# gnlpfjh/Scalable-E3-GNN

Measured on AMD Instinct MI355X. Metric: particles/sec (octree build + SEGNN fwd), 1M pts l_max=2, 1/2/4/8 MI355X, higher is better.
Workload: dtype f32; 1 GPU; 1000000 particles/GPU uniform in unit box, radius graph k~24 (E=23519616), SEGNN l_max=2 4 layers H=32 f32 storage; particles_per_gpu=1000000, edges_per_gpu=23519616, hidden=32, layers=4, lmax=2, parallelism=single GPU

## Files before the change

### include/e3gnn.h

```cpp
#ifndef E3GNN_H
#define E3GNN_H

#include <stdint.h>

#ifdef __cplusplus
extern "C" {
#endif

#define E3GNN_ABI_VERSION 3

enum {
  E3_OK = 0,
  E3_ERR_INVALID_ARG = 1,
  E3_ERR_BAD_IRREPS = 2,
  E3_ERR_MISSING_WEIGHT = 3,
  E3_ERR_UNSUPPORTED = 4,
  E3_ERR_HIP = 5,
  E3_ERR_NO_DEVICE = 6
};

enum { E3_F32 = 0, E3_F64 = 1, E3_BF16 = 2 };

enum { E3_CLS_0E = 0, E3_CLS_0O = 1, E3_CLS_1E = 2, E3_CLS_1O = 3 };

// ... 107 lines not shown
                       int dtype, void* packed, void* stream);
int e3_tp_forward(const e3_tp_plan* plan, const void* in1, int64_t ld_in1, const void* in2, int64_t ld_in2,
                  const void* packed, void* out, int64_t ld_out, int64_t B, int dtype, const float* in_scale,
                  int exact, void* stream);
int e3_pow2_scale(const e3_tp_segment* segs, const int64_t* nrows, int nseg, int target_log2, float* out4,
                  void* stream);
int e3_add_pow2_scale(const float* h, const float* u, float* out, int64_t n, int target_log2, float* out4,
                      void* stream);
int e3_tp_forward_fused(const e3_tp_plan* plan, const e3_tp_segment* segs, int nseg,
                        const void* in2, int64_t ld_in2, const void* packed, void* out, int64_t ld_out,
                        int64_t B, int dtype, int gate, const float* in_scale, void* stream);
int e3_tp_forward_fused_epilogue(const e3_tp_plan* plan, const e3_tp_segment* segs, int nseg, const void* in2,
                                 int64_t ld_in2, const void* packed, void* out, int64_t ld_out, int64_t B, int dtype,
                                 int gate, const float* in_scale, const void* residual, int64_t ld_residual,
                                 float* out_scale4, int target_log2, void* stream);
int e3_tp_backward(const e3_tp_plan* plan, const void* in1, int64_t ld_in1, const void* in2, int64_t ld_in2,
                   const void* packed, const void* grad_out, int64_t ld_gout, void* grad_in1, int64_t ld_gin1,
                   void* grad_in2, int64_t ld_gin2, void* const grad_weights[6], int64_t B, int dtype, void* stream);
int e3_tp_backward_weights(const e3_tp_plan* plan, const void* in1, int64_t ld_in1, const void* in2, int64_t ld_in2,
                           const void* packed, const void* grad_out, int64_t ld_gout, void* const grad_weights[6],
                           int64_t B, int dtype, void* stream);
int e3_tp_backward_operands(const e3_tp_plan* plan, const void* in1, int64_t ld_in1, const void* in2, int64_t ld_in2,
                            const void* packed, const void* grad_out, int64_t ld_gout, void* const features[6],
                            void* const gout[6], int64_t B, int dtype, void* stream);
int e3_tp_backward_contract(const e3_tp_plan* plan, const void* in1, int64_t ld_in1, const void* in2, int64_t ld_in2,
                            void* const t[6], void* grad_in1, int64_t ld_gin1, void* grad_in2, int64_t ld_gin2,
                            int64_t B, int dtype, void* stream);
int e3_tp_fused_supported(const e3_tp_plan* plan, int gate);
const char* e3_tp_last_fused_kernel(void);
int e3_tp_forward_fused_scatter(const e3_tp_plan* plan, const e3_tp_segment* segs, int nseg,
// ... 50 lines not shown
```

### scalable-e3-gnn_amd/_lib.py

```python
from __future__ import annotations

import ctypes
import os
from ctypes import POINTER, c_char_p, c_int, c_int32, c_int64, c_void_p

_HERE = os.path.dirname(os.path.abspath(__file__))
LIB_PATH = os.path.join(_HERE, "lib", "libe3gnn_hip.so")

E3_OK = 0
E3_F32, E3_F64, E3_BF16 = 0, 1, 2
CLS_NAMES = ("l0e", "l0o", "l1e", "l1o")

_lib = None

VoidP4 = c_void_p * 4
Float3 = ctypes.c_float * 3


class HaloEntry(ctypes.Structure):
    _fields_ = [("lo", ctypes.c_float * 3), ("hi", ctypes.c_float * 3), ("shift", ctypes.c_float * 3)]


SIGNATURES = {
    "e3_abi_version": (c_int, []),
# ... 71 lines not shown
    "e3_gate_blocks_backward": (c_int, [c_void_p, c_int64, c_void_p, c_int64, c_void_p, c_int64, c_int64, c_int, c_int,
                                        POINTER(c_int32), POINTER(c_int32), c_void_p]),
    "e3_segment_sum_backward": (c_int, [c_void_p, c_int64, c_void_p, c_int64, c_int, c_void_p, c_int64, c_void_p]),
    "e3_pow2_scale": (c_int, [c_void_p, POINTER(c_int64), c_int, c_int, c_void_p, c_void_p]),
    "e3_add_pow2_scale": (c_int, [c_void_p, c_void_p, c_void_p, c_int64, c_int, c_void_p, c_void_p]),
    "e3_tp_backward": (c_int, [c_void_p, c_void_p, c_int64, c_void_p, c_int64, c_void_p, c_void_p, c_int64, c_void_p,
                               c_int64, c_void_p, c_int64, c_void_p * 6, c_int64, c_int, c_void_p]),
    "e3_tp_backward_weights": (c_int, [c_void_p, c_void_p, c_int64, c_void_p, c_int64, c_void_p, c_void_p, c_int64, c_void_p,
                                       c_int64, c_int, c_void_p]),
    "e3_tp_backward_operands": (c_int, [c_void_p, c_void_p, c_int64, c_void_p, c_int64, c_void_p, c_void_p, c_int64, c_void_p,
                                        c_void_p, c_int64, c_int, c_void_p]),
    "e3_tp_backward_contract": (c_int, [c_void_p, c_void_p, c_int64, c_void_p, c_int64, c_void_p, c_void_p, c_int64, c_void_p,
                                        c_int64, c_int64, c_int, c_void_p]),
    "e3_tp_forward_fused_epilogue": (c_int, [c_void_p, c_void_p, c_int, c_void_p, c_int64, c_void_p, c_void_p, c_int64,
                                             c_int64, c_int, c_int, c_void_p, c_void_p, c_int64, c_void_p, c_int, c_void_p]),
    "e3_tp_fused_supported": (c_int, [c_void_p, c_int]),
    "e3_tp_last_fused_kernel": (ctypes.c_char_p, []),
    "e3_tp_forward_fused_scatter": (c_int, [c_void_p, c_void_p, c_int, c_void_p, c_int64, c_void_p, c_void_p, c_void_p,
                                            c_int64, c_int64, c_int, c_int, c_void_p, c_void_p]),
    "e3_segment_sum_bf16": (c_int, [c_void_p, c_int64, c_void_p, c_int64, c_int, c_void_p, c_int64, c_void_p]),
    "e3_edge_geometry_l2": (c_int, [c_void_p, c_void_p, c_void_p, c_int64, c_void_p, c_void_p, c_void_p, c_void_p]),
    "e3_gate_blocks": (c_int, [c_void_p, c_int64, c_void_p, c_int64, c_int64, c_int, c_int, POINTER(c_int32),
                               POINTER(c_int32), c_void_p]),
    "e3_l1tp_backward": (c_int, [c_void_p, c_void_p, c_int64, c_void_p, c_int64, VoidP4, VoidP4, c_void_p, c_int64,
                                 c_void_p, c_int64, c_void_p, VoidP4, c_void_p, c_int64, c_int, c_void_p]),
}


def load():
    global _lib
# ... 94 lines not shown
```

### scalable-e3-gnn_amd/csrc/e3_tp.hip

```cpp
#include "e3_common.h"
#include "cg_tables.h"
#include "e3_tp_internal.h"

#include <algorithm>
#include <cstdlib>
#include <map>
#include <mutex>
#include <utility>

namespace e3 {

static int tp_ensure_dyn_lds(const void* fn, size_t bytes) {
  if (bytes <= 64 * 1024) return E3_OK;
  static std::mutex mu;
  static std::map<std::pair<const void*, int>, size_t> have;
  int dev = 0;
  if (hipGetDevice(&dev) != hipSuccess) return E3_ERR_HIP;
  std::lock_guard<std::mutex> lock(mu);
  size_t& cur = have[std::make_pair(fn, dev)];
  if (bytes > cur) {
    if (hipFuncSetAttribute(fn, hipFuncAttributeMaxDynamicSharedMemorySize, (int)bytes) != hipSuccess) return E3_ERR_HIP;
    cur = bytes;
  }
  return E3_OK;
// ... 1112 lines not shown
  if ((dtype != E3_F32 && dtype != E3_BF16) || !plan->fast.usable || ld2 == 0) return E3_ERR_UNSUPPORTED;
  hipStream_t s = (hipStream_t)stream;
  if (out_scale4) E3_HIP_CHECK(hipMemsetAsync(out_scale4, 0, 16, s));
  if (B > 0) {
    if (!in2 || !packed || !out || ld2 < plan->dev.Dy) return E3_ERR_INVALID_ARG;
    int st = tp_ensure_device(plan);
    if (st != E3_OK) return st;
    st = fast_forward(&plan->fast, segs, nseg, plan->dev.D1, in2, ld2, (const char*)packed + fast_section_offset(plan), out,
                      ldo, B, gate, dtype, plan->dev.ocol, in_scale, s, nullptr, residual, ld_residual,
                      out_scale4 ? reinterpret_cast<uint32_t*>(out_scale4) + 2 : nullptr);
    if (st != E3_OK) return st;
  }
  return out_scale4 ? scale_finalize(out_scale4, target_log2, s) : E3_OK;
}

int e3_tp_forward_fused_scatter(const e3_tp_plan* plan, const e3_tp_segment* segs, int nseg, const void* in2,
                                int64_t ld2, const void* packed, const int32_t* row_node, void* out_nodes,
                                int64_t ldo, int64_t B, int dtype, int gate, const float* in_scale, void* stream) {
  if (!plan || !segs || !row_node || B < 0) return E3_ERR_INVALID_ARG;
  if ((dtype != E3_F32 && dtype != E3_BF16) || !gate || !plan->fast.usable || ld2 == 0) return E3_ERR_UNSUPPORTED;
  if (B == 0) return E3_OK;
  if (!in2 || !packed || !out_nodes || ld2 < plan->dev.Dy) return E3_ERR_INVALID_ARG;
  int st = tp_ensure_device(plan);
  if (st != E3_OK) return st;
  return fast_forward(&plan->fast, segs, nseg, plan->dev.D1, in2, ld2, (const char*)packed + fast_section_offset(plan),
                      out_nodes, ldo, B, gate, dtype, plan->dev.ocol, in_scale, (hipStream_t)stream, row_node);
}

int e3_tp_backward(const e3_tp_plan* plan, const void* in1, int64_t ld1, const void* in2, int64_t ld2,
                   const void* packed, const void* grad_out, int64_t ldg, void* grad_in1, int64_t ldg1,
// ... 100 lines not shown
```

### scalable-e3-gnn_amd/csrc/e3_tp_internal.h

```cpp
#pragma once
#include "e3_common.h"

#include <array>
#include <vector>

namespace e3 {

struct TpPath { int c1, l1, l2, wrow; };

struct FChunk {
  int col, count, l1;
  int wblk[3][3];
  int S[2], rows_per[2], inv[2];
};
struct FDev {
  int Dout, Dy, nchunks, ntab, lsh;
  int M[3], NT[3], Mpad[3], ooff[3];
  int bfoff[3];
  int bftotal;
};
struct FPack { int l3, orig_row, count, wblk; };

struct TpFast {
  FDev dev;
// ... 16 lines not shown
              const int32_t* ocol_tab, hipStream_t s);
int fast_forward(const TpFast* F, const e3_tp_segment* segs, int nseg, int D1, const void* in2, int64_t ld2,
                 const void* packed, void* out, int64_t ldo, int64_t B, int gate, int dtype, const int32_t* ocol_tab,
                 const float* in_scale, hipStream_t s, const int32_t* scatter = nullptr, const void* residual = nullptr,
                 int64_t ldr = 0, uint32_t* amax = nullptr);
int scale_finalize(float* out4, int target_log2, hipStream_t s);

void fast_note_kernel(const char* name);
const char* fast_last_kernel();

bool fast_gate_shape_ok(const TpFast* F);
bool r16_supported(const TpFast* F);
int fast_forward_r16(const TpFast* F, const void* seg_args, const void* in2, int64_t ld2, const void* packed, void* out,
                     int64_t ldo, int64_t B, int gate, int io16, const int32_t* ocol_tab, const float* in_scale,
                     hipStream_t s);

}
```

### scalable-e3-gnn_amd/csrc/e3_tp_mfma.hip

```cpp
#include "e3_common.h"
#include "e3_tp_internal.h"

#include <algorithm>
#include <cstdlib>
#include <vector>

namespace e3 {

#include "e3_tp_mfma_core.h"

template <typename T>
__global__ void fast_absmax_kernel(const T* w0, int64_t n0, const T* w1, int64_t n1, const T* w2, int64_t n2,
                                   uint32_t* hdr) {
  const T* w[3] = {w0, w1, w2};
  const int64_t n[3] = {n0, n1, n2};
  float m = 0.f;
  for (int c = 0; c < 3; ++c)
    for (int64_t i = blockIdx.x * (int64_t)blockDim.x + threadIdx.x; i < n[c]; i += (int64_t)gridDim.x * blockDim.x)
      m = fmax_finite(m, to_acc(w[c][i]));
  for (int o = 32; o > 0; o >>= 1) m = fmaxf(m, __shfl_xor(m, o));
  if ((threadIdx.x & 63) == 0 && m > 0.f) atomicMax(hdr, __builtin_bit_cast(uint32_t, m));
}

template <typename T>
// ... 148 lines not shown
  } else {
    hipLaunchKernelGGL(fast_absmax_kernel<float>, dim3(64), dim3(256), 0, s, (const float*)w[0], rows[0] * d.M[0],
                       (const float*)w[3], rows[1] * d.M[1], (const float*)w[4], rows[2] * d.M[2], hdr);
    hipLaunchKernelGGL(fast_pack_kernel<float>, grid, dim3(256), 0, s, (const float*)w[0], (const float*)w[3],
                       (const float*)w[4], (const float*)(n ? n[0] : nullptr), (const float*)(n ? n[3] : nullptr),
                       (const float*)(n ? n[4] : nullptr), (float*)packed, d, F->d_pack, npk, ocol_tab);
  }
  E3_HIP_CHECK(hipGetLastError());
  return E3_OK;
}

static thread_local const char* g_last_kernel = "";
void fast_note_kernel(const char* name) { g_last_kernel = name; }
const char* fast_last_kernel() { return g_last_kernel; }

int fast_forward(const TpFast* F, const e3_tp_segment* segs, int nseg, int D1, const void* in2, int64_t ld2,
                 const void* packed, void* out, int64_t ldo, int64_t B, int gate, int dtype, const int32_t* ocol_tab,
                 const float* in_scale, hipStream_t s, const int32_t* scatter, const void* residual, int64_t ldr,
                 uint32_t* amax) {
  if (!F->usable) return E3_ERR_UNSUPPORTED;
  const bool io16 = dtype == E3_BF16;
  const FDev& d = F->dev;
  if (nseg < 1 || nseg > 4) return E3_ERR_INVALID_ARG;
  SegArgs sa;
  int col = 0;
  if (ldo >= ((int64_t)1 << 24)) return E3_ERR_UNSUPPORTED;
  for (int i = 0; i < 4; ++i) { sa.base[i] = nullptr; sa.ld[i] = 0; sa.index[i] = nullptr; }
  for (int i = 0; i < nseg; ++i) {
    if (!segs[i].base || segs[i].ncols <= 0 || segs[i].ld < segs[i].ncols) return E3_ERR_INVALID_ARG;
    if (segs[i].ld >= (int64_t)1 << 29) return E3_ERR_UNSUPPORTED;
    sa.base[i] = segs[i].base;
    sa.ld[i] = segs[i].ld;
    sa.index[i] = segs[i].row_index;
    sa.col0[i] = col;
    col += segs[i].ncols;
  }
  for (int i = nseg; i < 5; ++i) sa.col0[i] = col;
  sa.nseg = nseg;
  sa.scatter = scatter;
  sa.residual = residual;
  sa.ldr = ldr;
  sa.amax = amax;
  if (residual && ldr >= (int64_t)1 << 29) return E3_ERR_UNSUPPORTED;
  if (col != D1) return E3_ERR_INVALID_ARG;
  for (auto& ch : F->h_chunks) {
    int cw = ch.count * (2 * ch.l1 + 1), sidx = 0;
    while (sidx + 1 < nseg && ch.col >= sa.col0[sidx + 1]) ++sidx;
    if (ch.col + cw > sa.col0[sidx + 1]) return E3_ERR_INVALID_ARG;
  }
  if (gate && !fast_gate_shape_ok(F)) return E3_ERR_UNSUPPORTED;
  const int r = fast_forward_r16(F, &sa, in2, ld2, packed, out, ldo, B, gate, io16 ? 1 : 0, ocol_tab, in_scale, s);
  if (r == 1) return E3_OK;
  return r < 0 ? -r : E3_ERR_UNSUPPORTED;
}

}
```

### scalable-e3-gnn_amd/csrc/e3_tp_mfma_r16.hip

```cpp
#include "e3_common.h"
#include "cg_tables.h"
#include "e3_tp_internal.h"

#include <algorithm>
#include <cstdlib>
#include <mutex>
#include <type_traits>
#include <utility>
#include <vector>

namespace e3 {

#include "e3_tp_mfma_core.h"

template <int NT16, bool IO16, int STRIDE>
__device__ __forceinline__ void mma_group(const uint4 (&ah)[NT16], const uint4 (&al)[IO16 ? 1 : NT16], const uint4 bh,
                                          const uint4 bl, f32x4* acc) {
  if constexpr (IO16) {
#pragma unroll
    for (int t = 0; t < NT16; ++t)
      acc[t * STRIDE] = mfma16(__builtin_bit_cast(bf16x8, ah[t]), __builtin_bit_cast(bf16x8, bh), acc[t * STRIDE]);
  } else {
#pragma unroll
    for (int t = 0; t < NT16; ++t)
// ... 491 lines not shown
#pragma unroll
      for (int t = 0; t < NT1; ++t) tile(I3{}, 1, t, [&](int q, int c) { return a1[2 * t + (q >> 2)][c][q & 3]; });
#pragma unroll
      for (int t = 0; t < NT2; ++t) tile(I5{}, 2, t, [&](int q, int c) { return a2[2 * t + (q >> 2)][c][q & 3]; });
    }
  }
  if constexpr (!SCAT) {
    if (segs.amax) {
#pragma unroll
      for (int o = 32; o > 0; o >>= 1) amax = fmaxf(amax, __shfl_xor(amax, o, 64));
      if (lane == 0 && amax > 0.f) atomicMax(segs.amax, __builtin_bit_cast(uint32_t, amax));
    }
  }
}

struct R16KernelEntry {
  int lsh, nt0, nt1, nt2;
  std::vector<int> l1s;
  const void* fn[2][2];
  const void* fn_scat;
};
#define E3_R16(LSH, a, b, c, SC, ...)                                                                          \
  {LSH, a, b, c, {__VA_ARGS__},                                                                                \
   {{(const void*)tp_fwd_mfma_r16_kernel<LSH, a, b, c, false, 1, false, __VA_ARGS__>,                           \
     (const void*)tp_fwd_mfma_r16_kernel<LSH, a, b, c, true, 1, false, __VA_ARGS__>},                           \
    {(const void*)tp_fwd_mfma_r16_kernel<LSH, a, b, c, false, 2, false, __VA_ARGS__>,                           \
     (const void*)tp_fwd_mfma_r16_kernel<LSH, a, b, c, true, 2, false, __VA_ARGS__>}},                          \
   SC ? (const void*)tp_fwd_mfma_r16_kernel<LSH, a, b, c, true, 1, SC, __VA_ARGS__> : nullptr}
static const std::vector<R16KernelEntry>& r16_kernels() {
  static const std::vector<R16KernelEntry> k = {
// ... 72 lines not shown
    }
  }
  const int64_t ntiles = (B + 15) / 16;
  const int grid = (int)std::min<int64_t>((ntiles + kR16Waves - 1) / kR16Waves, 256 * r16_waves_per_simd(d.NT[0], d.NT[1], d.NT[2]));
  const float* in2f = (const float*)in2;
  const float* pk = (const float*)packed;
  void* outf = out;
  const FDev* dd = F->d_dev;
  const FChunk* dc = F->d_chunks;
  void* args[] = {const_cast<void*>(sa_), &in2f, &ld2, &pk, &outf, &ldo, &B, &dd, &dc, &ocol_tab, &in_scale};
  if (hipLaunchKernel(fn, dim3(grid), dim3(64 * kR16Waves), args, lds_bytes, s) != hipSuccess) return -E3_ERR_HIP;
  fast_note_kernel("e3::tp_fwd_mfma_r16_kernel");
  return 1;
}

}
```

### scalable-e3-gnn_amd/segnn.py

```python
from __future__ import annotations

import torch
from torch import nn

from . import ops
from .irreps import Irreps
from .l1_tensor_prod import L1TensorProduct
from .message import FusedMessage
from .radius_graph import RadiusGraph
from .tensor_product import SHTensorProduct


def _hidden_irreps(H: int, lmax: int):
    hid = Irreps(f"{H}x0e+{H}x1o" + (f"+{H}x2e" if lmax == 2 else ""))
    gated = Irreps(f"{H}x0e+{lmax * H}x0e+{H}x1o" + (f"+{H}x2e" if lmax == 2 else ""))
    return hid, gated


def _make_tp(in_irreps, out_irreps, lmax: int):
    if lmax == 1:
        if Irreps(in_irreps).lmax == 1 and Irreps(out_irreps).lmax == 1:
            return L1TensorProduct(in_irreps, out_irreps)
        return SHTensorProduct(in_irreps, out_irreps, lmax_sh=1)
    return SHTensorProduct(in_irreps, out_irreps, lmax_sh=2)
# ... 78 lines not shown
            if self.fuse_scatter:
                a = self.msg2.forward_fused([(m, None)], Y, gate=True, scatter=(g.dst, g.rowptr.numel() - 1))
            if a is None:
                m = self.msg2.forward_fused([(m, None)], Y, gate=True)
                a = ops.segment_sum(m, g)
        else:
            m = ops.gather_concat(h, g, d)
            m = self._gate(self.msg1(m, Y))
            m = self._gate(self.msg2(m, Y))
            a = ops.segment_sum(m, g)
        if r16u:
            sc = None
            if f32 and h_scale is not None and halo is None:
                sc = ops.join_pow2_scales(h_scale, ops.pow2_scale([a]))
            if self.upd2.fused_supported(False) and h.stride(-1) == 1:
                u, u_scale = self.upd1.forward_fused([(h, None), (a, None)], A, gate=True, in_scale=sc,
                                                     out_scale=10 if f32 else None) if f32 else \
                    (self.upd1.forward_fused([(h, None), (a, None)], A, gate=True), None)
                if f32:
                    return self.upd2.forward_fused([(u, None)], A, gate=False, in_scale=u_scale, residual=h, out_scale=10)
                return self.upd2.forward_fused([(u, None)], A, gate=False, residual=h), None
            u = self.upd1.forward_fused([(h, None), (a, None)], A, gate=True, in_scale=sc)
        else:
            u = self._gate(self.upd1(torch.cat([h, a], 1), A))
        u = self.upd2(u, A)
        if f32 and inference:
            return ops.add_pow2_scale(h, u)
        return h + u, None


# ... 45 lines not shown
```

### scalable-e3-gnn_amd/tensor_product.py

```python
from __future__ import annotations

import ctypes
from math import sqrt

import torch
from torch import nn

from . import _lib, profiling
from .irreps import Irreps, as_blocks

CLASSES = ("l0e", "l0o", "l1e", "l1o", "l2e", "l2o")


class TPSegment(ctypes.Structure):
    _fields_ = [("base", ctypes.c_void_p), ("ld", ctypes.c_int64), ("row_index", ctypes.c_void_p),
                ("ncols", ctypes.c_int32), ("reserved", ctypes.c_int32)]


class TPPlan:

    def __init__(self, in1_irreps, out_irreps, lmax_sh):
        lib = _lib.load()
        self._blocks = ([tuple(b) for b in as_blocks(in1_irreps)], int(lmax_sh), [tuple(b) for b in as_blocks(out_irreps)])
        self._plans = _lib.DevicePlans("e3_tp_plan_create", "e3_tp_plan_destroy", *self._blocks)
# ... 158 lines not shown
            else:
                _lib.check(lib.e3_tp_forward_fused(h, ctypes.byref(segs), len(segments), in2.data_ptr(),
                                                   in2.stride(0), packed.data_ptr(), out.data_ptr(), out.stride(0), B,
                                                   _lib.dtype_code(io), 1 if gate else 0, sc, stream), "e3_tp_forward_fused")
            if t0 is not None:
                nb = sum((t.shape[0] * t.shape[1] * esz + (4 * B if idx is not None else 0)) for t, idx in
                         [(k, s[1]) for k, s in zip(keep, segments)]) + 4 * self.in2_dim * B + \
                     (esz * width * B if scatter is None else 4 * B + 4 * width * scatter[1])
                mode = "<bf16 storage, bf16 MFMA>" if io == torch.bfloat16 else "<fp16x3 split MFMA>"
                profiling.end(f"tp_fused{'+segsum' if scatter is not None else ''} {tag} B={B}", B, nb, t0, flops=self.flops_per_row * B,
                              kernel=(lib.e3_tp_last_fused_kernel() or b"e3::tp_fwd_mfma_r16_kernel").decode() + mode)
        if out_scale is not None:
            return out, sc4
        return out


def _rebuild_tpplan(in_blocks, lmax_sh, out_blocks):
    return TPPlan(in_blocks, out_blocks, lmax_sh)


_BWD_WORKSPACE_BYTES = 1 << 30
_BWD_GEMM_MIN_ROWS = 512


_WGRAD_SLAB = 4096
_BWD_FUSED_WGRAD = True


def _wgrad_accumulate(gw, F, G):
    R = F.shape[0]
# ... 132 lines not shown
        ns = [getattr(self, "norm_" + c) for c in CLASSES]
        return ws, ns

    def _packed_weights(self, dtype, device):
        ws, ns = self._tensors()
        return self._plan.packed(ws, ns, dtype, device)

    def fused_supported(self, gate: bool) -> bool:
        return self._plan.fused_supported(gate)

    def forward_fused(self, segments, in2, gate: bool = False, scatter=None, in_scale=None, residual=None, out_scale=None):
        ws, ns = self._tensors()
        return self._plan.forward_fused(ws, ns, segments, in2, gate, tag=f"{self.iri1}->{self.iro}", scatter=scatter,
                                        in_scale=in_scale, residual=residual, out_scale=out_scale)

    def forward(self, in1: torch.Tensor, in2: torch.Tensor) -> torch.Tensor:
        torch._assert(in1.shape[-1] == self.in1_dim,
                      f"Incorrect last dimension for in1 = {in1.shape[-1]}, required is {self.in1_dim}")
        torch._assert(in2.shape[-1] == self.in2_dim,
                      f"Incorrect last dimension for in2 = {in2.shape[-1]}, required is {self.in2_dim}")
        if not in1.is_cuda:
            raise RuntimeError("SHTensorProduct runs on ROCm tensors only; there is no CPU path")
        if torch.is_grad_enabled() and (in1.requires_grad or in2.requires_grad or
                                        any(p.requires_grad for p in self.parameters())):
            if in1.dtype not in (torch.float32, torch.float64):
                raise NotImplementedError("SHTensorProduct backward: float32 / float64 only")
            if in1.stride(-1) != 1:
                in1 = in1.contiguous()
            if in2.stride(-1) != 1:
                in2 = in2.contiguous()
# ... 38 lines not shown
```

Measured before the change: 10.79 million particles/s.

## Fuse node-update tensor-product pair into a single MFMA kernel

New measurement: 11.01 million particles/s (median of 6 runs). 2.0% higher.

```diff
diff --git a/include/e3gnn.h b/include/e3gnn.h
--- a/include/e3gnn.h
+++ b/include/e3gnn.h
@@ -145,6 +145,10 @@
                                  int64_t ld_in2, const void* packed, void* out, int64_t ld_out, int64_t B, int dtype,
                                  int gate, const float* in_scale, const void* residual, int64_t ld_residual,
                                  float* out_scale4, int target_log2, void* stream);
+int e3_tp_forward_update_pair(const e3_tp_plan* plan1, const e3_tp_plan* plan2, const e3_tp_segment* segs, int nseg,
+                              const void* in2, int64_t ld_in2, const void* packed1, const void* packed2,
+                              const float* in_scale, const void* residual, int64_t ld_residual, void* out,
+                              int64_t ld_out, int64_t B, int dtype, float* out_scale4, int target_log2, void* stream);
 int e3_tp_backward(const e3_tp_plan* plan, const void* in1, int64_t ld_in1, const void* in2, int64_t ld_in2,
                    const void* packed, const void* grad_out, int64_t ld_gout, void* grad_in1, int64_t ld_gin1,
                    void* grad_in2, int64_t ld_gin2, void* const grad_weights[6], int64_t B, int dtype, void* stream);
diff --git a/scalable-e3-gnn_amd/_lib.py b/scalable-e3-gnn_amd/_lib.py
--- a/scalable-e3-gnn_amd/_lib.py
+++ b/scalable-e3-gnn_amd/_lib.py
@@ -109,6 +109,9 @@
                                         c_int64, c_int64, c_int, c_void_p]),
     "e3_tp_forward_fused_epilogue": (c_int, [c_void_p, c_void_p, c_int, c_void_p, c_int64, c_void_p, c_void_p, c_int64,
                                              c_int64, c_int, c_int, c_void_p, c_void_p, c_int64, c_void_p, c_int, c_void_p]),
+    "e3_tp_forward_update_pair": (c_int, [c_void_p, c_void_p, c_void_p, c_int, c_void_p, c_int64, c_void_p, c_void_p,
+                                          c_void_p, c_void_p, c_int64, c_void_p, c_int64, c_int64, c_int, c_void_p, c_int,
+                                          c_void_p]),
     "e3_tp_fused_supported": (c_int, [c_void_p, c_int]),
     "e3_tp_last_fused_kernel": (ctypes.c_char_p, []),
     "e3_tp_forward_fused_scatter": (c_int, [c_void_p, c_void_p, c_int, c_void_p, c_int64, c_void_p, c_void_p, c_void_p,
diff --git a/scalable-e3-gnn_amd/csrc/e3_tp.hip b/scalable-e3-gnn_amd/csrc/e3_tp.hip
--- a/scalable-e3-gnn_amd/csrc/e3_tp.hip
+++ b/scalable-e3-gnn_amd/csrc/e3_tp.hip
@@ -1150,6 +1150,30 @@
   return out_scale4 ? scale_finalize(out_scale4, target_log2, s) : E3_OK;
 }
 
+int e3_tp_forward_update_pair(const e3_tp_plan* plan1, const e3_tp_plan* plan2, const e3_tp_segment* segs, int nseg,
+                              const void* in2, int64_t ld2, const void* packed1, const void* packed2,
+                              const float* in_scale, const void* residual, int64_t ld_residual, void* out, int64_t ldo,
+                              int64_t B, int dtype, float* out_scale4, int target_log2, void* stream) {
+  if (!plan1 || !plan2 || !segs || B < 0 || (residual && ld_residual <= 0)) return E3_ERR_INVALID_ARG;
+  if (out_scale4 && (target_log2 < -20 || target_log2 > 14)) return E3_ERR_INVALID_ARG;
+  if ((dtype != E3_F32 && dtype != E3_BF16) || ld2 == 0 || !e3::r16_pair_supported(&plan1->fast, &plan2->fast))
+    return E3_ERR_UNSUPPORTED;
+  if (!in2 || !packed1 || !packed2 || !out || ld2 < plan1->dev.Dy || ldo < plan2->dev.Dout) return E3_ERR_INVALID_ARG;
+  hipStream_t s = (hipStream_t)stream;
+  int st = tp_ensure_device(plan1);
+  if (st == E3_OK) st = tp_ensure_device(plan2);
+  if (st != E3_OK) return st;
+  if (out_scale4) E3_HIP_CHECK(hipMemsetAsync(out_scale4, 0, 16, s));
+  if (B > 0) {
+    st = fast_forward_pair(&plan1->fast, &plan2->fast, segs, nseg, plan1->dev.D1, in2, ld2,
+                           (const char*)packed1 + fast_section_offset(plan1), (const char*)packed2 + fast_section_offset(plan2),
+                           out, ldo, B, dtype, plan1->dev.ocol, plan2->dev.ocol, in_scale, residual, ld_residual,
+                           out_scale4 ? reinterpret_cast<uint32_t*>(out_scale4) + 2 : nullptr, s);
+    if (st != E3_OK) return st;
+  }
+  return out_scale4 ? scale_finalize(out_scale4, target_log2, s) : E3_OK;
+}
+
 int e3_tp_forward_fused_scatter(const e3_tp_plan* plan, const e3_tp_segment* segs, int nseg, const void* in2,
                                 int64_t ld2, const void* packed, const int32_t* row_node, void* out_nodes,
                                 int64_t ldo, int64_t B, int dtype, int gate, const float* in_scale, void* stream) {
diff --git a/scalable-e3-gnn_amd/csrc/e3_tp_internal.h b/scalable-e3-gnn_amd/csrc/e3_tp_internal.h
--- a/scalable-e3-gnn_amd/csrc/e3_tp_internal.h
+++ b/scalable-e3-gnn_amd/csrc/e3_tp_internal.h
@@ -54,5 +54,13 @@
 int fast_forward_r16(const TpFast* F, const void* seg_args, const void* in2, int64_t ld2, const void* packed, void* out,
                      int64_t ldo, int64_t B, int gate, int io16, const int32_t* ocol_tab, const float* in_scale,
                      hipStream_t s);
+bool r16_pair_supported(const TpFast* F1, const TpFast* F2);
+int fast_forward_pair_r16(const TpFast* F1, const TpFast* F2, const void* seg_args, const void* in2, int64_t ld2,
+                          const void* packed1, const void* packed2, void* out, int64_t ldo, int64_t B, int io16,
+                          const int32_t* ocol1, const int32_t* ocol2, const float* in_scale, hipStream_t s);
+int fast_forward_pair(const TpFast* F1, const TpFast* F2, const e3_tp_segment* segs, int nseg, int D1, const void* in2,
+                      int64_t ld2, const void* packed1, const void* packed2, void* out, int64_t ldo, int64_t B, int dtype,
+                      const int32_t* ocol1, const int32_t* ocol2, const float* in_scale, const void* residual,
+                      int64_t ldr, uint32_t* amax, hipStream_t s);
 
 }
diff --git a/scalable-e3-gnn_amd/csrc/e3_tp_mfma.hip b/scalable-e3-gnn_amd/csrc/e3_tp_mfma.hip
--- a/scalable-e3-gnn_amd/csrc/e3_tp_mfma.hip
+++ b/scalable-e3-gnn_amd/csrc/e3_tp_mfma.hip
@@ -186,15 +186,9 @@
 void fast_note_kernel(const char* name) { g_last_kernel = name; }
 const char* fast_last_kernel() { return g_last_kernel; }
 
-int fast_forward(const TpFast* F, const e3_tp_segment* segs, int nseg, int D1, const void* in2, int64_t ld2,
-                 const void* packed, void* out, int64_t ldo, int64_t B, int gate, int dtype, const int32_t* ocol_tab,
-                 const float* in_scale, hipStream_t s, const int32_t* scatter, const void* residual, int64_t ldr,
-                 uint32_t* amax) {
-  if (!F->usable) return E3_ERR_UNSUPPORTED;
-  const bool io16 = dtype == E3_BF16;
-  const FDev& d = F->dev;
+static int fast_seg_args(const TpFast* F, const e3_tp_segment* segs, int nseg, int D1, int64_t ldo, const int32_t* scatter,
+                         const void* residual, int64_t ldr, uint32_t* amax, SegArgs& sa) {
   if (nseg < 1 || nseg > 4) return E3_ERR_INVALID_ARG;
-  SegArgs sa;
   int col = 0;
   if (ldo >= ((int64_t)1 << 24)) return E3_ERR_UNSUPPORTED;
   for (int i = 0; i < 4; ++i) { sa.base[i] = nullptr; sa.ld[i] = 0; sa.index[i] = nullptr; }
@@ -220,10 +214,36 @@
     while (sidx + 1 < nseg && ch.col >= sa.col0[sidx + 1]) ++sidx;
     if (ch.col + cw > sa.col0[sidx + 1]) return E3_ERR_INVALID_ARG;
   }
+  return E3_OK;
+}
+
+int fast_forward(const TpFast* F, const e3_tp_segment* segs, int nseg, int D1, const void* in2, int64_t ld2,
+                 const void* packed, void* out, int64_t ldo, int64_t B, int gate, int dtype, const int32_t* ocol_tab,
+                 const float* in_scale, hipStream_t s, const int32_t* scatter, const void* residual, int64_t ldr,
+                 uint32_t* amax) {
+  if (!F->usable) return E3_ERR_UNSUPPORTED;
+  const bool io16 = dtype == E3_BF16;
+  SegArgs sa;
+  const int st = fast_seg_args(F, segs, nseg, D1, ldo, scatter, residual, ldr, amax, sa);
+  if (st != E3_OK) return st;
   if (gate && !fast_gate_shape_ok(F)) return E3_ERR_UNSUPPORTED;
   const int r = fast_forward_r16(F, &sa, in2, ld2, packed, out, ldo, B, gate, io16 ? 1 : 0, ocol_tab, in_scale, s);
   if (r == 1) return E3_OK;
   return r < 0 ? -r : E3_ERR_UNSUPPORTED;
 }
 
-}
+int fast_forward_pair(const TpFast* F1, const TpFast* F2, const e3_tp_segment* segs, int nseg, int D1, const void* in2,
+                      int64_t ld2, const void* packed1, const void* packed2, void* out, int64_t ldo, int64_t B, int dtype,
+                      const int32_t* ocol1, const int32_t* ocol2, const float* in_scale, const void* residual,
+                      int64_t ldr, uint32_t* amax, hipStream_t s) {
+  if (!F1->usable || !F2->usable || !r16_pair_supported(F1, F2)) return E3_ERR_UNSUPPORTED;
+  SegArgs sa;
+  const int st = fast_seg_args(F1, segs, nseg, D1, ldo, nullptr, residual, ldr, amax, sa);
+  if (st != E3_OK) return st;
+  const int r = fast_forward_pair_r16(F1, F2, &sa, in2, ld2, packed1, packed2, out, ldo, B, dtype == E3_BF16 ? 1 : 0,
+                                      ocol1, ocol2, in_scale, s);
+  if (r == 1) return E3_OK;
+  return r < 0 ? -r : E3_ERR_UNSUPPORTED;
+}
+
+}
diff --git a/scalable-e3-gnn_amd/csrc/e3_tp_mfma_r16.hip b/scalable-e3-gnn_amd/csrc/e3_tp_mfma_r16.hip
--- a/scalable-e3-gnn_amd/csrc/e3_tp_mfma_r16.hip
+++ b/scalable-e3-gnn_amd/csrc/e3_tp_mfma_r16.hip
@@ -529,6 +529,347 @@
   }
 }
 
+struct PairArgs {
+  const float* packed;
+  const FDev* dp;
+  const FChunk* chunks;
+  const int32_t* ocol_tab;
+};
+constexpr int kPairTarget = 10;
+
+template <int LSH, int NT0, int NT1, int NT2, int MODE, int... L1S>
+__global__ __launch_bounds__(256, 2) void tp_update_pair_r16_kernel(SegArgs segs, const float* __restrict__ in2, int64_t ld2,
+                                                                    const float* __restrict__ packed,
+                                                                    void* __restrict__ outv, int64_t ldo, int64_t B,
+                                                                    const FDev* __restrict__ dp,
+                                                                    const FChunk* __restrict__ chunks,
+                                                                    const int32_t* __restrict__ ocol_tab,
+                                                                    const float* __restrict__ in_scale, PairArgs pr) {
+  constexpr bool IO16 = MODE == 2;
+  constexpr int NL = (NT1 > 0 ? 1 : 0) + (NT2 > 0 ? 1 : 0);
+  static_assert(NT1 == 1 && NT2 <= 1 && NT0 == 1 + NL, "hidden 32: scalars and one gate block per degree, one tile each");
+  constexpr int CHUNK = r16_chunk(r16_max({L1S...}), NL);
+  extern __shared__ __align__(16) unsigned char smem_raw[];
+  float* lds = reinterpret_cast<float*>(smem_raw);
+  const int tid = threadIdx.x, lane = tid & 63;
+  const int wave = __builtin_amdgcn_readfirstlane(tid >> 6);
+  const int nwaves = blockDim.x >> 6;
+  const int j = lane & 15, g = lane >> 4;
+  const int Dout = dp->Dout, Dy = dp->Dy, nchunks = dp->nchunks, ntab = dp->ntab;
+  const int Dout2 = pr.dp->Dout, ntab2 = pr.dp->ntab;
+  int cMpad[3], cOoff[3], cBfoff[3], cM2[3], cMpad2[3], cOoff2[3], cBfoff2[3];
+#pragma unroll
+  for (int c = 0; c < 3; ++c) {
+    cMpad[c] = dp->Mpad[c]; cOoff[c] = dp->ooff[c]; cBfoff[c] = dp->bfoff[c];
+    cM2[c] = pr.dp->M[c]; cMpad2[c] = pr.dp->Mpad[c]; cOoff2[c] = pr.dp->ooff[c]; cBfoff2[c] = pr.dp->bfoff[c];
+  }
+
+  float* nrm = lds;
+  int* ocl = reinterpret_cast<int*>(nrm + ((Dout + 15) & ~15));
+  float* nrm2 = reinterpret_cast<float*>(ocl + ((ntab + 15) & ~15));
+  int* ocl2 = reinterpret_cast<int*>(nrm2 + ((Dout2 + 15) & ~15));
+  float* cbuf = reinterpret_cast<float*>(ocl2 + ((ntab2 + 15) & ~15)) + (size_t)wave * (CHUNK + 160);
+  float* ybuf = cbuf + CHUNK;
+  const float* hdr = packed + ((Dout + 3) & ~3);
+  const float* hdr2 = pr.packed + ((Dout2 + 3) & ~3);
+  const float xs = (!IO16 && in_scale) ? in_scale[0] : 1.0f;
+  const float unscale = IO16 ? 1.0f : hdr[2] * (in_scale ? in_scale[1] : 1.0f);
+  const float unscale2 = IO16 ? 1.0f : hdr2[2];
+  for (int i = tid; i < Dout; i += blockDim.x) nrm[i] = packed[i] * unscale;
+  for (int i = tid; i < ntab; i += blockDim.x) ocl[i] = ocol_tab[i];
+  for (int i = tid; i < Dout2; i += blockDim.x) nrm2[i] = pr.packed[i] * unscale2;
+  for (int i = tid; i < ntab2; i += blockDim.x) ocl2[i] = pr.ocol_tab[i];
+  __syncthreads();
+  const uint4* whi_base = reinterpret_cast<const uint4*>(hdr + 4);
+  const uint4* wlo_base = reinterpret_cast<const uint4*>(hdr + 4 + (dp->bftotal >> 1));
+  const uint4* whi2_base = reinterpret_cast<const uint4*>(hdr2 + 4);
+  const uint4* wlo2_base = reinterpret_cast<const uint4*>(hdr2 + 4 + (pr.dp->bftotal >> 1));
+
+  const int64_t ntiles = (B + 15) / 16;
+  const int64_t tstride = (int64_t)gridDim.x * nwaves;
+  const int inv_dy = (65536 + Dy - 1) / Dy;
+  using Slots = PathSlots<LSH, NT0, NT1, NT2>;
+  using Slots2 = PathSlots<LSH, 1, NT1, NT2>;
+  using Seq = IntSeq<L1S...>;
+  using I0 = std::integral_constant<int, 0>;
+  using I1 = std::integral_constant<int, 1>;
+  using I2 = std::integral_constant<int, 2>;
+  using I3 = std::integral_constant<int, 3>;
+  using I5 = std::integral_constant<int, 5>;
+  auto chan_of = [&](int q) { return 16 * (q >> 2) + 4 * g + (q & 3); };
+  const bool out_vec = !(ldo & 3) && ((reinterpret_cast<uintptr_t>(outv) & 15) == 0) &&
+                       (!segs.residual || (!(segs.ldr & 3) && (reinterpret_cast<uintptr_t>(segs.residual) & 15) == 0));
+  float amax = 0.f;
+
+  for (int64_t tile = (int64_t)blockIdx.x * nwaves + wave; tile < ntiles; tile += tstride) {
+    const int64_t row0 = tile * 16;
+    const int nrows = (int)((B - row0) < 16 ? (B - row0) : 16);
+
+    auto stage = [&](int ci) {
+      const FChunk ch = chunks[ci];
+      const int s = (segs.nseg > 1 && ch.col >= segs.col0[1]) + (segs.nseg > 2 && ch.col >= segs.col0[2]) +
+                    (segs.nseg > 3 && ch.col >= segs.col0[3]);
+      auto pick = [&](auto v0, auto v1, auto v2, auto v3) {
+        auto v = v0;
+        v = s == 1 ? v1 : v;
+        v = s == 2 ? v2 : v;
+        v = s == 3 ? v3 : v;
+        return v;
+      };
+      const int64_t ld = pick(segs.ld[0], segs.ld[1], segs.ld[2], segs.ld[3]);
+      const char* base = reinterpret_cast<const char*>(pick(segs.base[0], segs.base[1], segs.base[2], segs.base[3]));
+      const int segcol = ch.col - pick(segs.col0[0], segs.col0[1], segs.col0[2], segs.col0[3]);
+      constexpr int ESZ = IO16 ? 2 : 4, EPU = 16 / ESZ, MI = IO16 ? 1 : 0;
+      const int cw = ch.count * (2 * ch.l1 + 1);
+      const int S = ch.S[MI], rows_per = ch.rows_per[MI];
+      const int rl = (lane * ch.inv[MI]) >> 16, u = lane - rl * S;
+      const bool lane_ok = rl < rows_per && u < cw / EPU;
+      const char* lsrc = base + ((row0 + rl) * ld + segcol) * ESZ + u * 16;
+      for (int r0 = 0; r0 < 16; r0 += rows_per)
+        if (lane_ok && r0 + rl < nrows)
+          __builtin_amdgcn_global_load_lds((glb_void_t*)(lsrc + (int64_t)r0 * ld * ESZ), (lds_void_t*)(cbuf + r0 * S * 4), 16,
+                                           0, 0);
+      for (int e = nrows * S * 4 + lane; e < 16 * S * 4; e += 64) cbuf[e] = 0.f;
+    };
+
+    for (int h = 0; h * 64 < 16 * Dy; ++h) {
+      const int e = h * 64 + lane;
+      const int yr = (e * inv_dy) >> 16, yc = e - yr * Dy;
+      if (e < 16 * Dy) {
+        if (yr < nrows)
+          __builtin_amdgcn_global_load_lds((glb_void_t*)(in2 + (row0 + yr) * ld2 + yc), (lds_void_t*)(ybuf + h * 64), 4,
+                                           0, 0);
+        else
+          ybuf[e] = 0.f;
+      }
+    }
+    stage(0);
+
+    f32x4 a0[2 * NT0][1], a1[2][3], a2[NT2 > 0 ? 2 : 1][5];
+#pragma unroll
+    for (int t = 0; t < 2 * NT0; ++t) a0[t][0] = f32x4{0, 0, 0, 0};
+#pragma unroll
+    for (int t = 0; t < 2; ++t)
+#pragma unroll
+      for (int c = 0; c < 3; ++c) a1[t][c] = f32x4{0, 0, 0, 0};
+#pragma unroll
+    for (int t = 0; t < (NT2 > 0 ? 2 : 1); ++t)
+#pragma unroll
+      for (int c = 0; c < 5; ++c) a2[t][c] = f32x4{0, 0, 0, 0};
+    float y[9];
+    int ci = 0;
+    auto process = [&](auto itag) {
+      constexpr int L1 = Seq::at(decltype(itag)::value);
+      wait_vm0();
+      wave_sync_lds();
+      if (ci == 0) {
+#pragma unroll
+        for (int q = 0; q < 9; ++q) y[q] = (q < Dy) ? ybuf[j * Dy + q] : 0.f;
+      }
+      const FChunk ch = chunks[ci];
+      float x[8][2 * L1 + 1];
+      load_x16<L1, IO16>(cbuf + j * (((32 * (2 * L1 + 1) / (IO16 ? 8 : 4)) | 1) * 4), g, xs, x);
+#define E3_RUN(L2v, L3v, ACC, NTv)                                                                             \
+  if constexpr (Slots::valid(L1, L2v, L3v)) {                                                                  \
+    const size_t o = (size_t)(cBfoff[L3v] >> 3) + (size_t)(2 * ch.wblk[L2v][L3v] + g) * cMpad[L3v] + j;        \
+    run16<L1, L2v, L3v, 2 * NTv, IO16>(x, true, whi_base + o, wlo_base + o, y, ACC);                            \
+  }
+      E3_RUN(0, 0, a0, NT0) E3_RUN(1, 0, a0, NT0) E3_RUN(2, 0, a0, NT0)
+      E3_RUN(0, 1, a1, NT1) E3_RUN(1, 1, a1, NT1) E3_RUN(2, 1, a1, NT1)
+      E3_RUN(0, 2, a2, NT2) E3_RUN(1, 2, a2, NT2) E3_RUN(2, 2, a2, NT2)
+#undef E3_RUN
+      wave_sync_lds();
+      if (ci + 1 < nchunks) stage(ci + 1);
+      ++ci;
+    };
+    for_each_index(process, std::make_index_sequence<sizeof...(L1S)>{});
+    wait_vm0();
+    wave_sync_lds();
+
+    {
+      const float* nrm0 = nrm + ocl[cOoff[0]];
+#pragma unroll
+      for (int q = 0; q < 8; ++q) {
+        const float s = a0[q >> 2][0][q & 3] * nrm0[chan_of(q)];
+        a0[q >> 2][0][q & 3] = s * sigmoid_(s);
+      }
+      const float* nv1 = nrm + ocl[cOoff[1]];
+#pragma unroll
+      for (int q = 0; q < 8; ++q) {
+        const float gq = sigmoid_(a0[2 + (q >> 2)][0][q & 3] * nrm0[32 + chan_of(q)]);
+#pragma unroll
+        for (int c = 0; c < 3; ++c) a1[q >> 2][c][q & 3] = (gq * a1[q >> 2][c][q & 3]) * nv1[3 * chan_of(q) + c];
+      }
+      if constexpr (NT2 > 0) {
+        const float* nv2 = nrm + ocl[cOoff[2]];
+#pragma unroll
+        for (int q = 0; q < 8; ++q) {
+          const float gq = sigmoid_(a0[4 + (q >> 2)][0][q & 3] * nrm0[64 + chan_of(q)]);
+#pragma unroll
+          for (int c = 0; c < 5; ++c) a2[q >> 2][c][q & 3] = (gq * a2[q >> 2][c][q & 3]) * nv2[5 * chan_of(q) + c];
+        }
+      }
+    }
+    float srow = 1.0f, isrow = 1.0f;
+    if constexpr (!IO16) {
+      float m = 0.f;
+#pragma unroll
+      for (int q = 0; q < 8; ++q) {
+        m = fmax_finite(m, a0[q >> 2][0][q & 3]);
+#pragma unroll
+        for (int c = 0; c < 3; ++c) m = fmax_finite(m, a1[q >> 2][c][q & 3]);
+        if constexpr (NT2 > 0) {
+#pragma unroll
+          for (int c = 0; c < 5; ++c) m = fmax_finite(m, a2[q >> 2][c][q & 3]);
+        }
+      }
+      m = fmaxf(m, __shfl_xor(m, 16, 64));
+      m = fmaxf(m, __shfl_xor(m, 32, 64));
+      srow = pow2_scale_from_bits(__builtin_bit_cast(uint32_t, m), kPairTarget);
+      isrow = 1.0f / srow;
+    }
+
+    f32x4 b0[2][1], b1[2][3], b2[NT2 > 0 ? 2 : 1][5];
+#pragma unroll
+    for (int t = 0; t < 2; ++t) {
+      b0[t][0] = f32x4{0, 0, 0, 0};
+#pragma unroll
+      for (int c = 0; c < 3; ++c) b1[t][c] = f32x4{0, 0, 0, 0};
+    }
+#pragma unroll
+    for (int t = 0; t < (NT2 > 0 ? 2 : 1); ++t)
+#pragma unroll
+      for (int c = 0; c < 5; ++c) b2[t][c] = f32x4{0, 0, 0, 0};
+    auto put = [&](auto dtag, auto val) {
+      constexpr int D = decltype(dtag)::value;
+      if constexpr (IO16) {
+        uint16_t* o16 = reinterpret_cast<uint16_t*>(cbuf) + j * (8 * (((32 * D) / 8) | 1));
+#pragma unroll
+        for (int q = 0; q < 8; ++q)
+#pragma unroll
+          for (int c = 0; c < D; ++c) o16[D * chan_of(q) + c] = __builtin_bit_cast(uint16_t, (__bf16)val(q, c));
+      } else {
+#pragma unroll
+        for (int q = 0; q < 8; ++q)
+#pragma unroll
+          for (int c = 0; c < D; ++c) cbuf[j * (32 * D + 4) + D * chan_of(q) + c] = val(q, c) * srow;
+      }
+      wave_sync_lds();
+    };
+    auto mul2 = [&](auto ltag) {
+      constexpr int L1 = decltype(ltag)::value;
+      const FChunk ch = pr.chunks[L1];
+      float x[8][2 * L1 + 1];
+      load_x16<L1, IO16>(cbuf + j * (((32 * (2 * L1 + 1) / (IO16 ? 8 : 4)) | 1) * 4), g, 1.0f, x);
+#define E3_RUN2(L2v, L3v, ACC, NTv)                                                                            \
+  if constexpr (Slots2::valid(L1, L2v, L3v)) {                                                                 \
+    const size_t o = (size_t)(cBfoff2[L3v] >> 3) + (size_t)(2 * ch.wblk[L2v][L3v] + g) * cMpad2[L3v] + j;      \
+    run16<L1, L2v, L3v, 2 * NTv, IO16>(x, true, whi2_base + o, wlo2_base + o, y, ACC);                          \
+  }
+      E3_RUN2(0, 0, b0, 1) E3_RUN2(1, 0, b0, 1) E3_RUN2(2, 0, b0, 1)
+      E3_RUN2(0, 1, b1, NT1) E3_RUN2(1, 1, b1, NT1) E3_RUN2(2, 1, b1, NT1)
+      E3_RUN2(0, 2, b2, NT2) E3_RUN2(1, 2, b2, NT2) E3_RUN2(2, 2, b2, NT2)
+#undef E3_RUN2
+      wave_sync_lds();
+    };
+    put(I1{}, [&](int q, int) { return a0[q >> 2][0][q & 3]; });
+    mul2(I0{});
+    put(I3{}, [&](int q, int c) { return a1[q >> 2][c][q & 3]; });
+    mul2(I1{});
+    if constexpr (NT2 > 0) {
+      put(I5{}, [&](int q, int c) { return a2[q >> 2][c][q & 3]; });
+      mul2(I2{});
+    }
+
+    float* ot = cbuf;
+    auto emit = [&](auto dtag, const int l3, auto val) {
+      constexpr int D = decltype(dtag)::value;
+      constexpr int TS = 32 * D + 4;
+      constexpr int UPR = 32 * D / 4;
+      const int base = cOoff2[l3];
+      const int cnt = cM2[l3] < 32 ? cM2[l3] : 32;
+      const int width = cnt * D;
+      auto col = [&](int lc) { return ocl2[base + lc / D] + lc % D; };
+      const int colb = col(0);
+      const bool vec = out_vec && ocl2[base + cnt - 1] == colb + (cnt - 1) * D && !(colb & 3) && !(width & 3);
+#pragma unroll
+      for (int q = 0; q < 8; ++q)
+#pragma unroll
+        for (int c = 0; c < D; ++c) ot[j * TS + D * chan_of(q) + c] = val(q, c);
+      wave_sync_lds();
+      if (vec) {
+        constexpr uint32_t INV = (65536 + UPR - 1) / UPR;
+        static_assert(((16u * UPR - 1) * INV >> 16) == 15 && ((15u * UPR) * INV >> 16) == 15 &&
+                      ((14u * UPR + UPR - 1) * INV >> 16) == 14, "reciprocal");
+        const uint32_t ldo32 = (uint32_t)ldo;
+#pragma unroll 2
+        for (int it = 0; it < UPR / 4; ++it) {
+          const uint32_t u = it * 64 + lane;
+          const uint32_t row = __umul24(u, INV) >> 16, un = u - __umul24(row, UPR);
+          const uint32_t lc0 = un * 4;
+          float4 v = *reinterpret_cast<const float4*>(ot + __umul24(row, TS) + un * 4);
+          const float* np = nrm2 + colb + lc0;
+          const float n0 = np[0], n1 = np[1], n2 = np[2], n3 = np[3];
+          if ((int)row < nrows && (int)lc0 < width) {
+            v.x *= n0; v.y *= n1; v.z *= n2; v.w *= n3;
+            const uint32_t o = __umul24(row, ldo32) + (uint32_t)colb + lc0;
+            if (segs.residual) {
+              const int64_t ro = (row0 + row) * segs.ldr + colb + lc0;
+              if (IO16) {
+                const uint2 rk = *reinterpret_cast<const uint2*>(reinterpret_cast<const uint16_t*>(segs.residual) + ro);
+                v.x += __builtin_bit_cast(float, rk.x << 16); v.y += __builtin_bit_cast(float, rk.x & 0xffff0000u);
+                v.z += __builtin_bit_cast(float, rk.y << 16); v.w += __builtin_bit_cast(float, rk.y & 0xffff0000u);
+              } else {
+                const float4 rv = *reinterpret_cast<const float4*>(reinterpret_cast<const float*>(segs.residual) + ro);
+                v.x += rv.x; v.y += rv.y; v.z += rv.z; v.w += rv.w;
+              }
+            }
+            amax = fmax_finite4(amax, v);
+            if (IO16) {
+              uint2 pk;
+              pk.x = __builtin_bit_cast(uint32_t, __builtin_convertvector(f32x2_t{v.x, v.y}, bf16x2_t));
+              pk.y = __builtin_bit_cast(uint32_t, __builtin_convertvector(f32x2_t{v.z, v.w}, bf16x2_t));
+              *reinterpret_cast<uint2*>(reinterpret_cast<uint16_t*>(outv) + row0 * ldo + o) = pk;
+            } else {
+              *reinterpret_cast<float4*>(reinterpret_cast<float*>(outv) + row0 * ldo + o) = v;
+            }
+          }
+        }
+      } else {
+        for (int lc = lane; lc < 32 * D; lc += 64) {
+          if (lc >= width) continue;
+          const int64_t c0 = row0 * ldo + col(lc);
+          const float nv = nrm2[col(lc)];
+          const float* src = ot + lc;
+#pragma unroll 1
+          for (int r = 0; r < nrows; ++r) {
+            float v = src[r * TS] * nv;
+            if (segs.residual) {
+              const int64_t ro = (row0 + r) * segs.ldr + col(lc);
+              v += IO16 ? __builtin_bit_cast(float, (uint32_t)reinterpret_cast<const uint16_t*>(segs.residual)[ro] << 16)
+                        : reinterpret_cast<const float*>(segs.residual)[ro];
+            }
+            amax = fmax_finite(amax, v);
+            if (IO16)
+              reinterpret_cast<uint16_t*>(outv)[c0 + (int64_t)r * ldo] = __builtin_bit_cast(uint16_t, (__bf16)v);
+            else
+              reinterpret_cast<float*>(outv)[c0 + (int64_t)r * ldo] = v;
+          }
+        }
+      }
+      wave_sync_lds();
+    };
+    emit(I1{}, 0, [&](int q, int) { return b0[q >> 2][0][q & 3] * isrow; });
+    emit(I3{}, 1, [&](int q, int c) { return b1[q >> 2][c][q & 3] * isrow; });
+    if constexpr (NT2 > 0) emit(I5{}, 2, [&](int q, int c) { return b2[q >> 2][c][q & 3] * isrow; });
+  }
+  if (segs.amax) {
+#pragma unroll
+    for (int o = 32; o > 0; o >>= 1) amax = fmaxf(amax, __shfl_xor(amax, o, 64));
+    if (lane == 0 && amax > 0.f) atomicMax(segs.amax, __builtin_bit_cast(uint32_t, amax));
+  }
+}
+
 struct R16KernelEntry {
   int lsh, nt0, nt1, nt2;
   std::vector<int> l1s;
@@ -631,4 +972,87 @@
   return 1;
 }
 
-}
+struct R16PairEntry {
+  int lsh, nt0, nt1, nt2;
+  std::vector<int> l1s;
+  const void* fn[2];
+};
+#define E3_R16_PAIR(LSH, a, b, c, ...)                                                                         \
+  {LSH, a, b, c, {__VA_ARGS__},                                                                                \
+   {(const void*)tp_update_pair_r16_kernel<LSH, a, b, c, 1, __VA_ARGS__>,                                       \
+    (const void*)tp_update_pair_r16_kernel<LSH, a, b, c, 2, __VA_ARGS__>}}
+static const R16PairEntry* r16_pair_find(const TpFast* F1, const TpFast* F2) {
+  static const std::vector<R16PairEntry> k = {
+      E3_R16_PAIR(2, 3, 1, 1, 0, 1, 2, 0, 1, 2),
+  };
+  const FDev& d = F1->dev;
+  const FDev& d2 = F2->dev;
+  std::vector<int> l1s;
+  for (auto& c : F1->h_chunks) {
+    if (c.count != 32) return nullptr;
+    l1s.push_back(c.l1);
+  }
+  const int nu = 1 + (d.NT[1] > 0) + (d.NT[2] > 0);
+  if (!fast_gate_shape_ok(F1) || d.M[0] != 32 * nu) return nullptr;
+  if (d2.lsh != d.lsh || d2.Dy != d.Dy || (int)F2->h_chunks.size() != nu) return nullptr;
+  for (int l = 0; l < nu; ++l)
+    if (F2->h_chunks[l].l1 != l || F2->h_chunks[l].count != 32) return nullptr;
+  if (d2.NT[0] != 1 || d2.NT[1] != d.NT[1] || d2.NT[2] != d.NT[2]) return nullptr;
+  for (auto& e : k)
+    if (e.lsh == d.lsh && e.nt0 == d.NT[0] && e.nt1 == d.NT[1] && e.nt2 == d.NT[2] && e.l1s == l1s) return &e;
+  return nullptr;
+}
+static size_t r16_pair_lds_bytes(const TpFast* F1, const TpFast* F2, int nwaves) {
+  const FDev& d = F1->dev;
+  const FDev& d2 = F2->dev;
+  const size_t tables =
+      (size_t)(((d.Dout + 15) & ~15) + ((d.ntab + 15) & ~15) + ((d2.Dout + 15) & ~15) + ((d2.ntab + 15) & ~15)) * 4;
+  int lin = 0;
+  for (auto& c : F1->h_chunks) lin = std::max(lin, c.l1);
+  return tables + nwaves * (size_t)(r16_chunk(lin, d.NT[2] > 0 ? 2 : 1) + 160) * 4;
+}
+
+bool r16_pair_supported(const TpFast* F1, const TpFast* F2) {
+  return r16_find(F1) != nullptr && r16_pair_find(F1, F2) != nullptr && 2 * r16_pair_lds_bytes(F1, F2, kR16Waves) <= (size_t)kFastLds;
+}
+
+int fast_forward_pair_r16(const TpFast* F1, const TpFast* F2, const void* sa_, const void* in2, int64_t ld2,
+                          const void* packed1, const void* packed2, void* out, int64_t ldo, int64_t B, int io16,
+                          const int32_t* ocol1, const int32_t* ocol2, const float* in_scale, hipStream_t s) {
+  const SegArgs& sa = *static_cast<const SegArgs*>(sa_);
+  const R16PairEntry* e = r16_pair_find(F1, F2);
+  if (!e || sa.scatter) return 0;
+  const int epu = io16 ? 8 : 4;
+  for (int i = 0; i < sa.nseg; ++i)
+    if (sa.index[i] || (sa.ld[i] % epu) || ((sa.col0[i + 1] - sa.col0[i]) % epu) ||
+        (reinterpret_cast<uintptr_t>(sa.base[i]) & 15))
+      return 0;
+  const void* fn = e->fn[io16 ? 1 : 0];
+  const size_t lds_bytes = r16_pair_lds_bytes(F1, F2, kR16Waves);
+  if (2 * lds_bytes > (size_t)kFastLds) return 0;
+  {
+    int dev = 0;
+    if (hipGetDevice(&dev) != hipSuccess) return -E3_ERR_HIP;
+    static std::mutex mu;
+    static std::vector<std::pair<const void*, int>> configured;
+    std::lock_guard<std::mutex> lock(mu);
+    if (std::find(configured.begin(), configured.end(), std::make_pair(fn, dev)) == configured.end()) {
+      if (hipFuncSetAttribute(fn, hipFuncAttributeMaxDynamicSharedMemorySize, (int)lds_bytes) != hipSuccess) return -E3_ERR_HIP;
+      configured.emplace_back(fn, dev);
+    }
+  }
+  const int64_t ntiles = (B + 15) / 16;
+  const int grid = (int)std::min<int64_t>((ntiles + kR16Waves - 1) / kR16Waves, 256 * 2);
+  const float* in2f = (const float*)in2;
+  const float* pk = (const float*)packed1;
+  void* outf = out;
+  const FDev* dd = F1->d_dev;
+  const FChunk* dc = F1->d_chunks;
+  PairArgs pa{(const float*)packed2, F2->d_dev, F2->d_chunks, ocol2};
+  void* args[] = {const_cast<void*>(sa_), &in2f, &ld2, &pk, &outf, &ldo, &B, &dd, &dc, &ocol1, &in_scale, &pa};
+  if (hipLaunchKernel(fn, dim3(grid), dim3(64 * kR16Waves), args, lds_bytes, s) != hipSuccess) return -E3_ERR_HIP;
+  fast_note_kernel("e3::tp_update_pair_r16_kernel");
+  return 1;
+}
+
+}
diff --git a/scalable-e3-gnn_amd/segnn.py b/scalable-e3-gnn_amd/segnn.py
--- a/scalable-e3-gnn_amd/segnn.py
+++ b/scalable-e3-gnn_amd/segnn.py
@@ -116,6 +116,11 @@
             if f32 and h_scale is not None and halo is None:
                 sc = ops.join_pow2_scales(h_scale, ops.pow2_scale([a]))
             if self.upd2.fused_supported(False) and h.stride(-1) == 1:
+                if isinstance(self.upd1, SHTensorProduct) and a.stride(-1) == 1:
+                    r = self.upd1.forward_update_pair(self.upd2, [(h, None), (a, None)], A, in_scale=sc, residual=h,
+                                                      out_scale=10 if f32 else None)
+                    if r is not None:
+                        return r if f32 else (r, None)
                 u, u_scale = self.upd1.forward_fused([(h, None), (a, None)], A, gate=True, in_scale=sc,
                                                      out_scale=10 if f32 else None) if f32 else \
                     (self.upd1.forward_fused([(h, None), (a, None)], A, gate=True), None)
diff --git a/scalable-e3-gnn_amd/tensor_product.py b/scalable-e3-gnn_amd/tensor_product.py
--- a/scalable-e3-gnn_amd/tensor_product.py
+++ b/scalable-e3-gnn_amd/tensor_product.py
@@ -196,6 +196,52 @@
             return out, sc4
         return out
 
+    def forward_update_pair(self, ws, ns, plan2, ws2, ns2, segments, in2, in_scale=None, residual=None, out_scale=None):
+        lib = _lib.load()
+        B = in2.shape[0]
+        dev = in2.device
+        io = segments[0][0].dtype
+        if io not in (torch.float32, torch.bfloat16) or in2.dtype != torch.float32 or in2.stride(-1) != 1:
+            return None
+        segs = (TPSegment * len(segments))()
+        keep = []
+        for i, (t, idx) in enumerate(segments):
+            if idx is not None or t.dtype != io or t.stride(-1) != 1 or t.shape[0] != B:
+                return None
+            keep.append(t)
+            segs[i].base, segs[i].ld, segs[i].ncols = t.data_ptr(), t.stride(0), t.shape[1]
+        out = torch.empty((B, plan2.out_dim), dtype=io, device=dev)
+        if residual is not None and (residual.shape != out.shape or residual.dtype != io or residual.stride(-1) != 1):
+            raise RuntimeError(f"forward_update_pair: residual must be {tuple(out.shape)} {io}, contiguous rows")
+        with torch.cuda.device(dev):
+            h1, h2 = self.handle(dev), plan2.handle(dev)
+            packed1 = self.packed(ws, ns, io, dev)
+            packed2 = plan2.packed(ws2, ns2, io, dev)
+            if io == torch.float32 and in_scale is None:
+                from . import ops
+                in_scale = ops.pow2_scale(keep)
+            sc = in_scale.data_ptr() if (in_scale is not None and io == torch.float32) else None
+            sc4 = torch.empty(4, dtype=torch.float32, device=dev) if out_scale is not None else None
+            stream = torch.cuda.current_stream(dev).cuda_stream
+            t0 = profiling.begin() if profiling.enabled() else None
+            st = lib.e3_tp_forward_update_pair(
+                h1, h2, ctypes.byref(segs), len(segments), in2.data_ptr(), in2.stride(0), packed1.data_ptr(),
+                packed2.data_ptr(), sc, residual.data_ptr() if residual is not None else None,
+                residual.stride(0) if residual is not None else 0, out.data_ptr(), out.stride(0), B, _lib.dtype_code(io),
+                sc4.data_ptr() if sc4 is not None else None, int(out_scale) if out_scale is not None else 0, stream)
+            if st == 4:
+                return None
+            _lib.check(st, "e3_tp_forward_update_pair")
+            if t0 is not None:
+                esz = out.element_size()
+                nb = sum(t.numel() * esz for t in keep) + 4 * self.in2_dim * B + esz * out.numel() * (2 if residual is not None else 1)
+                mode = "<bf16 storage, bf16 MFMA>" if io == torch.bfloat16 else "<fp16x3 split MFMA>"
+                profiling.end(f"tp_update_pair B={B}", B, nb, t0, flops=(self.flops_per_row + plan2.flops_per_row) * B,
+                              kernel=(lib.e3_tp_last_fused_kernel() or b"e3::tp_update_pair_r16_kernel").decode() + mode)
+        if out_scale is not None:
+            return out, sc4
+        return out
+
 
 def _rebuild_tpplan(in_blocks, lmax_sh, out_blocks):
     return TPPlan(in_blocks, out_blocks, lmax_sh)
@@ -358,6 +404,12 @@
         return self._plan.forward_fused(ws, ns, segments, in2, gate, tag=f"{self.iri1}->{self.iro}", scatter=scatter,
                                         in_scale=in_scale, residual=residual, out_scale=out_scale)
 
+    def forward_update_pair(self, second, segments, in2, in_scale=None, residual=None, out_scale=None):
+        ws, ns = self._tensors()
+        ws2, ns2 = second._tensors()
+        return self._plan.forward_update_pair(ws, ns, second._plan, ws2, ns2, segments, in2, in_scale=in_scale,
+                                              residual=residual, out_scale=out_scale)
+
     def forward(self, in1: torch.Tensor, in2: torch.Tensor) -> torch.Tensor:
         torch._assert(in1.shape[-1] == self.in1_dim,
                       f"Incorrect last dimension for in1 = {in1.shape[-1]}, required is {self.in1_dim}")
```
